# sash-a/es_pytorch

Hardware: AMD Instinct MI355X
Metric: env-steps/sec (whole node), Humanoid-v2 objective-ES (higher is better)
Workload: dtype bf16; 1 GPU; model=MLP(256, 256), env=Humanoid-v2, global_batch=1280, policies_per_gen=1280, episode_len=1000, seq_len=1000, objective=reward, parallelism=dp1, pair_rollout=True, eps_encoding=e4m3, noise_table_elems=250000000, n_params=166673

## Files before the change

es_pytorch_amd/core/engine.py:

```python
from __future__ import annotations

import time
from typing import List, Optional, Tuple

import numpy as np
import torch

from es_pytorch_amd import ops
from es_pytorch_amd.core.noisetable import NoiseTable
from es_pytorch_amd.core.policy import Policy
from es_pytorch_amd.envs.base import BatchedEnv
from es_pytorch_amd.nn.obstat import ObStat
from es_pytorch_amd.nn.optimizers import SGD, Adam, Optimizer
from es_pytorch_amd.parallel.comm import Comm
from es_pytorch_amd.rollout.results import RewardResult
from es_pytorch_amd.utils.novelty import novelty_batch
from es_pytorch_amd.utils.rankers import CenteredRanker, Ranker


def forward_perm(dims: List[int]) -> torch.Tensor:
    perm = []
    flat_off = 0
    for I, O in zip(dims[:-1], dims[1:]):
        w = np.arange(O * I, dtype=np.int64).reshape(O, I)
        perm.append((flat_off + w.T).reshape(-1))
        flat_off += O * I
        perm.append(np.arange(O, dtype=np.int64) + flat_off)
        flat_off += O
    return torch.from_numpy(np.concatenate(perm))


class _NoiselessResult(RewardResult):

    def __init__(self, reward: float, position, steps: int, ob_shape):
        super().__init__([reward], [float(position[0]), float(position[1]),
                                    float(position[2])] * 2,
                         np.zeros((1,) + tuple(ob_shape)), steps)


class GpuEngine:
    def __init__(self, cfg, comm: Comm, policy: Policy, nt: NoiseTable, env: BatchedEnv,
                 rs: np.random.RandomState, objective: str = "reward",
                 use_graph: bool = True, novelty_k: int = 10,
                 fused: Optional[bool] = None, rollout_mode: str = "step",
                 split_dyn: Optional[bool] = None,
                 pair_rollout: Optional[bool] = None,
                 eps_fp8: Optional[bool] = None,
                 weights_dtype: Optional[str] = None):
        self.rollout_mode = rollout_mode
        if weights_dtype is None:
            weights_dtype = cfg.general.get("weights_dtype", "bf16")
        if weights_dtype not in ("bf16", "fp32"):
            raise ValueError(f"weights_dtype must be 'bf16' or 'fp32', got "
                             f"{weights_dtype!r}")
        self.weights_dtype = weights_dtype
        self.fp32 = weights_dtype == "fp32"
        if self.fp32:
            for flag, val in (("pair_rollout", pair_rollout), ("eps_fp8", eps_fp8),
                              ("split_dyn", split_dyn)):
                if val is True:
                    raise ValueError(
                        f"{flag}=True is not available with weights_dtype='fp32' "
                        f"(the fp32 mode runs per-member fp32 rows only)")
            ignored = [k for k in ("pair_rollout", "eps_fp8", "split_dyn")
                       if bool(cfg.general.get(k, False))]
            if ignored and comm.rank == 0:
                import sys
                print(f"[engine] weights_dtype=fp32: ignoring {', '.join(ignored)} "
                      f"from the config (no fp32 variant)", file=sys.stderr)
            pair_rollout = eps_fp8 = split_dyn = False
        self.steps_per_launch = int(cfg.general.get("steps_per_launch", 1) or 1)
        self.cfg = cfg
        self.comm = comm
        self.policy = policy
        self.nt = nt
        self.env = env
        self.rs = rs
        self.objective = objective
        self.device = nt.noise.device
        self.use_graph = use_graph and self.device.type == "cuda"
        self.novelty_k = novelty_k
        self.archive: Optional[torch.Tensor] = None

        ppg = cfg.general.policies_per_gen
        assert ppg % comm.size == 0 and (ppg / comm.size) % 2 == 0, \
            "policies_per_gen must split into antithetic pairs per rank"
        self.pairs = int(ppg // comm.size // 2)
        self.eps = max(1, int(cfg.general.get("eps_per_policy", 1) or 1))
        self.M = 2 * self.pairs + 1
        self.B = self.M * self.eps
        assert env.batch == self.B, f"env batch {env.batch} != engine batch {self.B}"

        self.dims = policy._module.layer_dims()
        if len(self.dims) - 1 > 8:
            raise ValueError(
                f"model has {len(self.dims) - 1} layers; the fused HIP forward "
                f"supports at most 8 (ES_MAXL in ops/csrc/hip/mlp_core.h) — "
                f"reduce policy.layer_sizes or raise ES_MAXL and rebuild")
        if max(self.dims) > 2048:
            raise ValueError(
                f"widest layer is {max(self.dims)}; the fused HIP forward "
                f"supports at most 2048 (ES_MAXDIM in ops/csrc/hip/mlp_core.h) "
                f"— narrow policy.layer_sizes or raise ES_MAXDIM and rebuild")
        self.bins = int(getattr(policy._module, "bins", 0))
# ... 53 lines not shown
        self.rew_total = torch.zeros(self.B, dtype=torch.float32, device=d)
        self.member_steps = torch.zeros(self.B, dtype=torch.float32, device=d)
        self.behv = torch.zeros((self.B, 3), dtype=torch.float32, device=d)
        self.save_mask = torch.zeros(self.B, dtype=torch.float32, device=d)
        self.ob_sum = torch.zeros(D, dtype=torch.float64, device=d)
        self.ob_sumsq = torch.zeros(D, dtype=torch.float64, device=d)
        self.ob_count = torch.zeros((), dtype=torch.float64, device=d)
        self.obs_buf = torch.zeros((self.B, D), dtype=torch.float32, device=d)

        self.max_steps = int(cfg.env.max_steps)
        self.gen = 0
        self._graph: Optional[torch.cuda.CUDAGraph] = None
        self.timings = {}
        self._side = torch.cuda.Stream(self.device) if self.device.type == "cuda" else None
        self._offs_prefetched = False

        from es_pytorch_amd.envs.locomotion import SyntheticLocomotion
        self.fused = (isinstance(env, SyntheticLocomotion) and self.device.type == "cuda"
                      if fused is None else bool(fused))
        if self.fused:
            self.mo_sum = torch.zeros((self.B, D), dtype=torch.float32, device=d)
            self.mo_sumsq = torch.zeros((self.B, D), dtype=torch.float32, device=d)

        self.dyn_group = int(cfg.general.get("dyn_group", 5) or 5)
        want_split = bool(cfg.general.get("split_dyn", False)) if split_dyn is None \
            else bool(split_dyn)
        self.split_dyn = (want_split and self.fused and env.sdim % 8 == 0
                          and env.ac_dim <= 64 and self.dyn_group in (2, 4, 5, 8))
        if self.split_dyn:
            self.act_scratch = torch.empty(self.B * 64, dtype=torch.float32, device=d)

        fp8_possible = (bool(cfg.general.get("eps_fp8", False))
                        if eps_fp8 is None else bool(eps_fp8)) and \
            self.rollout_mode == "step" and self.steps_per_launch == 1 and \
            self._fp8_layout_ok(self.dims)
        if pair_rollout is not None:
            want_pair = bool(pair_rollout)
        else:
            gate_blocks = 256 if fp8_possible else 384
            want_pair = (bool(cfg.general.get("pair_rollout", False))
                         and self.pairs * self.eps >= gate_blocks)
        self.pair_rollout = (want_pair and self.fused and not self.split_dyn
                             and self.pairs >= 1)
        self._zero_off = torch.zeros(1, dtype=torch.int64, device=d)
        self._zero_sign = torch.zeros(1, dtype=torch.float32, device=d)
        want_fp8 = (bool(cfg.general.get("eps_fp8", False))
                    if eps_fp8 is None else bool(eps_fp8))
        self.eps_fp8 = fp8_possible and self.pair_rollout
        if want_fp8 and not self.eps_fp8 and comm.rank == 0:
            import sys
            print("[engine] eps_fp8 requested but unavailable for this "
                  "model/path — using bf16 eps rows", file=sys.stderr)
        if self.pair_rollout:
            self._theta_blob = torch.empty((2, self.row_stride), dtype=torch.bfloat16,
                                           device=d)
            self.theta_row = self._theta_blob[:1]
            eps_dt = torch.uint8 if self.eps_fp8 else torch.bfloat16
            self._eps_blob = torch.empty((self.pairs + 1, self.row_stride),
                                         dtype=eps_dt, device=d)
            self.eps_rows = self._eps_blob[:self.pairs]
            self._zeros_n = torch.zeros(self.n, dtype=torch.float32, device=d)
            self._one_signs = torch.ones(self.pairs, dtype=torch.float32, device=d)
        self._warned_host_ranker = False

    @staticmethod
    def _fp8_layout_ok(dims: List[int]) -> bool:
        off = 0
        for I, O in zip(dims[:-1], dims[1:]):
            vec = (O % 8 == 0) and (off % 8 == 0)
            if vec and (off + (I % 2) * O) % 16 != 0:
                return False
            off += I * O + O
        return True

    def _grad_qstd(self) -> float:
        return float(self.policy.std) if self.eps_fp8 else 0.0

    @property
    def numerics(self) -> dict:
        if self.pair_rollout:
            path, enc = "pair", "e4m3" if self.eps_fp8 else "bf16"
# ... 104 lines not shown
            ops.check(ops.hip().es_loco_step(*common, self._stream()), "es_loco_step")

    def _loco_episode(self, member_base: int, n_members: int, noiseless_from: int,
                      n_steps: Optional[int] = None, salt_base: int = 0,
                      weights_ptr: Optional[int] = None, wrow0: int = 0,
                      block_threads: int = 256):
        env = self.env
        goal_ptr = env.goal.data_ptr() if env.goal_conditioned else None
        fn, name = (ops.hip().es_loco_episode_f32, "es_loco_episode_f32") \
            if self.fp32 else (ops.hip().es_loco_episode, "es_loco_episode")
        ops.check(fn(
            self.weights.data_ptr() if weights_ptr is None else weights_ptr,
            self.obmean.data_ptr(), self.obstd.data_ptr(),
            self.dims_arr.ctypes.data, len(self.dims_arr), self.seed_dev.data_ptr(),
            self.max_steps if n_steps is None else n_steps,
            float(self.policy._module.ob_clip),
            self.acstd_dev.data_ptr(), self.row_stride,
            env.s.data_ptr(), env.pos.data_ptr(), goal_ptr,
            env.A_bf16.data_ptr(), env.B.data_ptr(), env.b0.data_ptr(),
            env.wv.data_ptr(), env.wa.data_ptr(), env.wy.data_ptr(), env.wh.data_ptr(),
            self.alive.data_ptr(), self.rew_total.data_ptr(),
            self.member_steps.data_ptr(), self.behv.data_ptr(),
            self.mo_sum.data_ptr(), self.mo_sumsq.data_ptr(),
            member_base, n_members, salt_base, wrow0, env.sdim, env.ac_dim,
            int(env.goal_conditioned), int(env.terminate_on_fall), noiseless_from,
            self.bins, self.eps, self.act_mode,
            float(env.leak), float(env.ctrl_cost), float(env.alive_bonus),
            float(env.fall_threshold), float(env.dt), int(block_threads),
            self._stream()), name)

    def _loco_pair_episode(self, n_steps: Optional[int] = None, salt_base: int = 0):
        env = self.env
        goal_ptr = env.goal.data_ptr() if env.goal_conditioned else None
        ops.check(ops.hip().es_loco_pair_episode(
            self.theta_row.data_ptr(), self.eps_rows.data_ptr(),
            self.obmean.data_ptr(), self.obstd.data_ptr(),
            self.dims_arr.ctypes.data, len(self.dims_arr),
            self.seed_dev.data_ptr(),
            float(self.policy._module.ob_clip), self.acstd_dev.data_ptr(),
            self.row_stride,
            env.s.data_ptr(), env.pos.data_ptr(), goal_ptr,
            env.A_bf16.data_ptr(), env.B.data_ptr(), env.b0.data_ptr(),
            env.wv.data_ptr(), env.wa.data_ptr(), env.wy.data_ptr(),
            env.wh.data_ptr(),
            self.alive.data_ptr(), self.rew_total.data_ptr(),
            self.member_steps.data_ptr(), self.behv.data_ptr(),
            self.mo_sum.data_ptr(), self.mo_sumsq.data_ptr(),
            self.pairs, env.sdim, env.ac_dim, int(env.goal_conditioned),
            int(env.terminate_on_fall), (self.M - 1) * self.eps, self.bins,
            self.eps, self.act_mode,
            float(env.leak), float(env.ctrl_cost), float(env.alive_bonus),
            float(env.fall_threshold), float(env.dt),
            self.max_steps if n_steps is None else int(n_steps), int(salt_base),
            self._stream()), "es_loco_pair_episode")

    def _loco_noiseless_episode(self):
        if self.pair_rollout:
            self._loco_episode((self.M - 1) * self.eps, self.eps, 0,
                               weights_ptr=self.theta_row.data_ptr(),
                               wrow0=self.M - 1, block_threads=512)
        else:
            self._loco_episode((self.M - 1) * self.eps, self.eps, 0,
                               block_threads=512)

    def _step_body(self, t: int):
        a = self._forward(self.obs_buf, salt=t + 1)
        ob, rew, done = self.env.step(a)
        alive = self.alive
        self.rew_total.add_(rew * alive)
        self.member_steps.add_(alive)
        am = alive.bool().unsqueeze(1)
        self.behv.copy_(torch.where(am, self.env.positions, self.behv))
        w = alive * self.save_mask
        self.ob_sum.add_((ob * w.unsqueeze(1)).sum(0).double())
        self.ob_sumsq.add_((ob * ob * w.unsqueeze(1)).sum(0).double())
        self.ob_count.add_(w.sum().double())
        self.alive.mul_(1.0 - done.float())
        self.obs_buf.copy_(ob)

    def _rollout_body(self):
        if self.fused and self.rollout_mode == "episode":
            main = torch.cuda.current_stream(self.device)
            self._side.wait_stream(main)
            with torch.cuda.stream(self._side):
                self._loco_noiseless_episode()
            if self.pair_rollout:
                self._loco_pair_episode()
# ... 2 lines not shown
            main.wait_stream(self._side)
            return
        if self.fused:
            main = torch.cuda.current_stream(self.device)
            self._side.wait_stream(main)
            with torch.cuda.stream(self._side):
                self._loco_noiseless_episode()
            k = self.steps_per_launch
            if k > 1:
                mm = (self.M - 1) * self.eps
                for t0 in range(0, self.max_steps, k):
                    n = min(k, self.max_steps - t0)
                    if self.pair_rollout:
                        self._loco_pair_episode(n_steps=n, salt_base=t0)
                    else:
                        self._loco_episode(0, mm, mm, n_steps=n, salt_base=t0)
            else:
                for t in range(self.max_steps):
                    self._loco_step(t)
            main.wait_stream(self._side)
        else:
            for t in range(self.max_steps):
                self._step_body(t)

    def _rollout(self):
        body = self._loco_step if self.fused else self._step_body
        if self.use_graph:
            if self._graph is None:
                s = torch.cuda.Stream(self.device)
                s.wait_stream(torch.cuda.current_stream(self.device))
                with torch.cuda.stream(s):
                    for t in range(3):
                        body(t)
                    if self.fused:
                        self._loco_noiseless_episode()
                torch.cuda.current_stream(self.device).wait_stream(s)
                self._reset_rollout_state()
                self.obs_buf.copy_(self.env.reset(self._gen_seed()))
                self._graph = torch.cuda.CUDAGraph()
                with torch.cuda.graph(self._graph):
                    self._rollout_body()
            self._graph.replay()
            return
        self._rollout_body()

    def _reset_rollout_state(self):
        self.alive.fill_(1.0)
        self.rew_total.zero_()
        self.member_steps.zero_()
        self.behv.zero_()
        self.ob_sum.zero_()
        self.ob_sumsq.zero_()
        self.ob_count.zero_()
        if self.fused:
            self.mo_sum.zero_()
            self.mo_sumsq.zero_()

    def _gen_seed(self) -> int:
        return (self.gen * 1000003 + self.comm.rank * 7919) & 0x7FFFFFFF

    def _member_rewards(self) -> torch.Tensor:
        return self.rew_total.view(self.M, self.eps).mean(1)

    def _member_behv(self) -> torch.Tensor:
        return self.behv.view(self.M, self.eps, 3)[:, -1]

# ... 269 lines not shown
```

es_pytorch_amd/ops/__init__.py:

```python
from __future__ import annotations

import ctypes
import os
import subprocess
from typing import Optional

_DIR = os.path.dirname(os.path.abspath(__file__))
_CPU_SO = os.path.join(_DIR, "_cpu_ops.so")
_HIP_SO = os.environ.get("ES_HIP_SO", os.path.join(_DIR, "_hip_ops.so"))

_cpu_lib: Optional[ctypes.CDLL] = None
_hip_lib: Optional[ctypes.CDLL] = None


class _BuildLock:

    def __init__(self, path: str):
        self.path = path + ".lock"
        self._fl = None

    def __enter__(self):
        try:
            from filelock import FileLock
            self._fl = FileLock(self.path)
# ... 110 lines not shown

def _bind_hip(lib):
    u64, i64, u32, i32, f32, p = (ctypes.c_uint64, ctypes.c_int64, ctypes.c_uint32,
                                  ctypes.c_int32, ctypes.c_float, ctypes.c_void_p)
    lib.es_noise_fill.argtypes = [p, i64, u64, u32, p]
    lib.es_pheno_bf16.argtypes = [p, p, p, p, p, i64, i64, i64, f32, p]
    lib.es_pheno_fp8.argtypes = [p, p, p, p, i32, i64, i64, i64, f32, p]
    lib.es_mlp_fwd.argtypes = [p, p, p, p, p, p, i32, p, u64, i32, f32, p, i64, i32,
                               i32, i32, i32, i32, p, p, p]
    lib.es_grad_gather.argtypes = [p, p, p, p, i64, i64, f32, p]
    lib.es_adam_step.argtypes = [p, p, p, p, i64, f32, f32, f32, f32, f32, f32, p]
    lib.es_sgd_step.argtypes = [p, p, p, i64, f32, f32, f32, f32, p]
    lib.es_loco_step.argtypes = [p, p, p, p, i32, p, u64, f32, p, i64,
                                 p, p, p, p, p, p, p, p, p, p,
                                 p, p, p, p, p, p,
                                 i32, i32, i32, i32, i32, i32, i32, i32, i32,
                                 f32, f32, f32, f32, f32, p]
    lib.es_loco_step_split.argtypes = [p, p, p, p, i32, p, u64, f32, p, i64,
                                       p, p, p, p, p, p, p, p, p, p,
                                       p, p, p, p, p, p,
                                       i32, i32, i32, i32, i32, i32, i32, i32, i32,
                                       f32, f32, f32, f32, f32, p, i32, p]
    lib.es_loco_pair_step.argtypes = [p, p, p, p, p, i32, p, u64, f32, p, i64,
                                      p, p, p, p, p, p, p, p, p, p,
                                      p, p, p, p, p, p,
                                      i32, i32, i32, i32, i32, i32, i32, i32, i32,
                                      f32, f32, f32, f32, f32, p]
    lib.es_loco_pair_step_fp8.argtypes = lib.es_loco_pair_step.argtypes
    lib.es_loco_pair_episode.argtypes = [p, p, p, p, p, i32, p, f32, p, i64,
                                         p, p, p, p, p, p, p, p, p, p,
                                         p, p, p, p, p, p,
                                         i32, i32, i32, i32, i32, i32, i32, i32, i32,
                                         f32, f32, f32, f32, f32, i32, i32, p]
    lib.es_loco_episode.argtypes = [p, p, p, p, i32, p, i32, f32, p, i64,
                                    p, p, p, p, p, p, p, p, p, p,
                                    p, p, p, p, p, p,
                                    i32, i32, i32, i32, i32, i32, i32, i32, i32, i32,
                                    i32, i32, f32, f32, f32, f32, f32, i32, p]
    lib.es_pheno_f32.argtypes = lib.es_pheno_bf16.argtypes
    lib.es_mlp_fwd_f32.argtypes = lib.es_mlp_fwd.argtypes
    lib.es_loco_step_f32.argtypes = lib.es_loco_step.argtypes
    lib.es_loco_episode_f32.argtypes = lib.es_loco_episode.argtypes
    for fn in ["es_pheno_f32", "es_mlp_fwd_f32", "es_loco_step_f32",
               "es_loco_episode_f32",
               "es_noise_fill", "es_pheno_bf16", "es_pheno_fp8", "es_mlp_fwd",
               "es_grad_gather", "es_adam_step", "es_sgd_step", "es_loco_step",
               "es_loco_step_split", "es_loco_pair_step", "es_loco_pair_step_fp8",
               "es_loco_pair_episode", "es_loco_episode"]:
        getattr(lib, fn).restype = i32


def check(ret: int, name: str):
    if ret != 0:
        raise RuntimeError(f"HIP op {name} failed with hipError_t={ret}")
```

es_pytorch_amd/ops/csrc/hip/rollout_loco.hip:

```cpp
#include "mlp_core.h"

struct LocoArgs {
  int S;
  int A;
  int D;
  int goal;
  int terminate;
  int noiseless_from;
  int bins;
  int act_mode;
  int eps;
  int wrow0;
  float leak, ctrl, alive_bonus, fall_thr, dt, ob_clip;
  int64_t row_stride;
};

struct LocoPtrs {
  const uint16_t* weights;
  const float *obmean, *obstd, *ac_std_dev;
  const uint64_t* seed_dev;
  float *s_glob, *pos;
  const float *goal, *Bm, *b0, *wv, *wa, *wy, *wh;
  const uint16_t* Am;
  float *alive, *rew_total, *member_steps, *behv, *mo_sum, *mo_sumsq;
// ... 112 lines not shown
      for (; i + 11 * PART < S; i += step4) {
        const uint4 n0 = ld(i + 8 * PART), n1 = ld(i + 9 * PART),
                    n2 = ld(i + 10 * PART), n3 = ld(i + 11 * PART);
        bf8_fma(c0, raws[i], acc);
        bf8_fma(c1, raws[i + PART], acc);
        bf8_fma(c2, raws[i + 2 * PART], acc);
        bf8_fma(c3, raws[i + 3 * PART], acc);
        c0 = d0; c1 = d1; c2 = d2; c3 = d3;
        d0 = n0; d1 = n1; d2 = n2; d3 = n3;
      }
      if (i < S) bf8_fma(c0, raws[i], acc);
      if (i + PART < S) bf8_fma(c1, raws[i + PART], acc);
      if (i + 2 * PART < S) bf8_fma(c2, raws[i + 2 * PART], acc);
      if (i + 3 * PART < S) bf8_fma(c3, raws[i + 3 * PART], acc);
      if (i + 4 * PART < S) bf8_fma(d0, raws[i + 4 * PART], acc);
      if (i + 5 * PART < S) bf8_fma(d1, raws[i + 5 * PART], acc);
      if (i + 6 * PART < S) bf8_fma(d2, raws[i + 6 * PART], acc);
      if (i + 7 * PART < S) bf8_fma(d3, raws[i + 7 * PART], acc);
      i += 8 * PART;
    }
    for (; i < S; i += PART) bf8_fma(ld(i), raws[i], acc);
#pragma unroll
    for (int q = 0; q < 8; ++q) partial[(ip * OCT + oi) * 8 + q] = acc[q];
  }
  __syncthreads();
}

#define ES_DYN_BM_BT 16

struct LocoBook {
  float px, py, gx, gy, rew_total, member_steps, ms0, ms1, mq0, mq1;
};

template <int NM>
__device__ __forceinline__ void loco_dyn_finish_n(
    const LocoArgs& la, const LocoPtrs& P, const int* b, const float* const* raws,
    const float* const* abuf, float* const* part, int tid, int nth) {
  const int S = la.S, A = la.A;
  float w_alive[NM];
  float *sb[NM], *ms[NM], *mq[NM];
#pragma unroll
  for (int m = 0; m < NM; ++m) {
    w_alive[m] = P.alive[b[m]];
    sb[m] = P.s_glob + (int64_t)b[m] * S;
    ms[m] = P.mo_sum + (int64_t)b[m] * la.D;
    mq[m] = P.mo_sumsq + (int64_t)b[m] * la.D;
  }
  const int wid = tid >> 6;
  const bool book = (tid & 63) == 0 && wid < NM;
  int bme = b[0];
  float alive_me = w_alive[0];
  float *part_me = part[0], *ms_me = ms[0], *mq_me = mq[0];
#pragma unroll
  for (int m = 1; m < NM; ++m)
    if (wid == m) {
      bme = b[m]; alive_me = w_alive[m];
      part_me = part[m]; ms_me = ms[m]; mq_me = mq[m];
    }
  LocoBook bk = {};
  if (book) {
    bk.px = P.pos[(int64_t)bme * 3 + 0];
    bk.py = P.pos[(int64_t)bme * 3 + 1];
    bk.rew_total = P.rew_total[bme];
    bk.member_steps = P.member_steps[bme];
    if (la.goal) {
      bk.gx = P.goal[(int64_t)bme * 2 + 0];
      bk.gy = P.goal[(int64_t)bme * 2 + 1];
      if (alive_me > 0.0f) {
        bk.ms0 = ms_me[S]; bk.ms1 = ms_me[S + 1];
        bk.mq0 = mq_me[S]; bk.mq1 = mq_me[S + 1];
      }
    }
  }

  float p0[NM], p1[NM], p2[NM], p3[NM];
#pragma unroll
  for (int m = 0; m < NM; ++m) p0[m] = p1[m] = p2[m] = p3[m] = 0.0f;
  {
    const bool oct8 = (S % 8 == 0);
    const int OCT = S >> 3;
    const int PART = oct8 ? nth / OCT : 0;
    for (int o = tid; o < S; o += nth) {
      const float b0o = P.b0[o], wvo = P.wv[o], wyo = P.wy[o], who = P.wh[o];
      float mso[NM], mqo[NM];
#pragma unroll
      for (int m = 0; m < NM; ++m)
        if (w_alive[m] > 0.0f) {
          mso[m] = ms[m][o];
          mqo[m] = mq[m][o];
        }
      float p[NM];
#pragma unroll
      for (int m = 0; m < NM; ++m) p[m] = b0o;
      if (oct8) {
        const int oo = o >> 3, j = o & 7;
        for (int pp = 0; pp < PART; ++pp)
#pragma unroll
          for (int m = 0; m < NM; ++m) p[m] += part[m][(pp * OCT + oo) * 8 + j];
      } else {
        for (int i = 0; i < S; ++i) {
          const float a = bf2f(P.Am[(int64_t)i * S + o]);
#pragma unroll
          for (int m = 0; m < NM; ++m) p[m] = fmaf(raws[m][i], a, p[m]);
        }
      }
      const float* bcol = P.Bm + o;
      int k0 = 0;
      for (; k0 + ES_DYN_BM_BT <= A; k0 += ES_DYN_BM_BT) {
        float bv[ES_DYN_BM_BT];
#pragma unroll
        for (int u = 0; u < ES_DYN_BM_BT; ++u) bv[u] = bcol[(int64_t)(k0 + u) * S];
#pragma unroll
        for (int u = 0; u < ES_DYN_BM_BT; ++u)
#pragma unroll
          for (int m = 0; m < NM; ++m) p[m] = fmaf(abuf[m][k0 + u], bv[u], p[m]);
      }
      if (k0 < A) {
        float bv[ES_DYN_BM_BT];
#pragma unroll
        for (int u = 0; u < ES_DYN_BM_BT - 1; ++u)
          if (k0 + u < A) bv[u] = bcol[(int64_t)(k0 + u) * S];
#pragma unroll
        for (int u = 0; u < ES_DYN_BM_BT - 1; ++u)
          if (k0 + u < A) {
#pragma unroll
            for (int m = 0; m < NM; ++m) p[m] = fmaf(abuf[m][k0 + u], bv[u], p[m]);
          }
      }
#pragma unroll
      for (int m = 0; m < NM; ++m) {
        const float sn = (1.0f - la.leak) * raws[m][o] + la.leak * tanhf(p[m]);
        sb[m][o] = sn;
        p0[m] = fmaf(sn, wvo, p0[m]);
        p1[m] = fmaf(sn, wyo, p1[m]);
        p2[m] = fmaf(sn, who, p2[m]);
        if (w_alive[m] > 0.0f) {
          ms[m][o] = mso[m] + sn;
          mq[m][o] = mqo[m] + sn * sn;
        }
      }
    }
    for (int j = tid; j < A; j += nth) {
      const float waj = P.wa[j];
#pragma unroll
      for (int m = 0; m < NM; ++m) {
        p0[m] = fmaf(0.5f * abuf[m][j], waj, p0[m]);
        p3[m] = fmaf(abuf[m][j], abuf[m][j], p3[m]);
      }
    }
  }
#pragma unroll
  for (int off = 32; off > 0; off >>= 1) {
#pragma unroll
    for (int m = 0; m < NM; ++m) {
      p0[m] += __shfl_down(p0[m], off);
      p1[m] += __shfl_down(p1[m], off);
      p2[m] += __shfl_down(p2[m], off);
      p3[m] += __shfl_down(p3[m], off);
    }
  }
  __syncthreads();
  if ((tid & 63) == 0) {
#pragma unroll
    for (int m = 0; m < NM; ++m) {
      part[m][wid * 4 + 0] = p0[m];
// ... 15 lines not shown
    }
    const float alive_old = alive_me;
    float rew;
    if (la.goal) {
      const float rx = bk.gx - bk.px;
      const float ry = bk.gy - bk.py;
      const float inv = 1.0f / (sqrtf(rx * rx + ry * ry) + 1e-6f);
      rew = vfwd * rx * inv + vy * ry * inv - la.ctrl * asq + la.alive_bonus;
    } else {
      rew = vfwd - la.ctrl * asq + la.alive_bonus;
    }
    const float px = bk.px + la.dt * vfwd;
    const float py = bk.py + la.dt * vy;
    P.pos[(int64_t)bme * 3 + 0] = px;
    P.pos[(int64_t)bme * 3 + 1] = py;
    P.pos[(int64_t)bme * 3 + 2] = h;
    const float done = (la.terminate && h < la.fall_thr) ? 1.0f : 0.0f;
    P.rew_total[bme] = bk.rew_total + rew * alive_old;
    P.member_steps[bme] = bk.member_steps + alive_old;
    if (alive_old > 0.0f) {
      P.behv[(int64_t)bme * 3 + 0] = px;
      P.behv[(int64_t)bme * 3 + 1] = py;
      P.behv[(int64_t)bme * 3 + 2] = h;
    }
    P.alive[bme] = alive_old * (1.0f - done);
    if (la.goal && alive_old > 0.0f) {
      const float rel0 = (bk.gx - px) * 0.1f;
      const float rel1 = (bk.gy - py) * 0.1f;
      ms_me[S] = bk.ms0 + rel0;
      mq_me[S] = bk.mq0 + rel0 * rel0;
      ms_me[S + 1] = bk.ms1 + rel1;
      mq_me[S + 1] = bk.mq1 + rel1 * rel1;
    }
  }
  __syncthreads();
}

__device__ __forceinline__ void loco_dyn_finish(
    const LocoArgs& la, const LocoPtrs& P, int b, const float* raws,
    const float* abuf, float* partial, int tid, int nth) {
  const int bs[1] = {b};
  const float* const rs[1] = {raws};
  const float* const as[1] = {abuf};
  float* const ps[1] = {partial};
  loco_dyn_finish_n<1>(la, P, bs, rs, as, ps, tid, nth);
}

__device__ __forceinline__ void loco_dyn_finish_pair(
    const LocoArgs& la, const LocoPtrs& P, int bp, int bm, const float* rawsP,
    const float* rawsM, const float* abufP, const float* abufM, float* partP,
    float* partM, int tid, int nth) {
  const int bs[2] = {bp, bm};
  const float* const rs[2] = {rawsP, rawsM};
  const float* const as[2] = {abufP, abufM};
  float* const ps[2] = {partP, partM};
  loco_dyn_finish_n<2>(la, P, bs, rs, as, ps, tid, nth);
}

template <typename WT = uint16_t>
__device__ __forceinline__ void loco_step_body(
    const MlpShape& sh, const LocoArgs& la, const LocoPtrs& P, int b, uint64_t salt,
    float* bufA, float* bufB, float* partial, float* raws, float* abuf) {
  loco_fwd_body<WT>(sh, la, P, b, salt, bufA, bufB, partial, raws, abuf);
  if (la.S % 8 == 0)
    loco_dyn_partials(P.Am, la.S, raws, partial, threadIdx.x, blockDim.x);
  loco_dyn_finish(la, P, b, raws, abuf, partial, threadIdx.x, blockDim.x);
}

#define ES_LOCO_CARVE(NTH)                                       \
  extern __shared__ __attribute__((aligned(16))) char smem[];    \
  float* bufA = reinterpret_cast<float*>(smem);                  \
  float* bufB = bufA + sh.maxdim;                                \
  float* partial = bufB + sh.maxdim;                             \
  float* raws = partial + (NTH) * 8;                             \
  float* abuf = raws + ((la.S + 3) & ~3);

__global__ void __launch_bounds__(256)
loco_step_kernel(MlpShape sh, LocoArgs la, LocoPtrs P, uint64_t salt) {
  ES_LOCO_CARVE(256);
  loco_step_body(sh, la, P, blockIdx.x, salt, bufA, bufB, partial, raws, abuf);
}

__global__ void __launch_bounds__(256)
loco_episode_kernel(MlpShape sh, LocoArgs la, LocoPtrs P, int member_base, int n_steps,
                    int salt_base) {
  ES_LOCO_CARVE(256);
  const int b = member_base + blockIdx.x;
  for (int t = 1; t <= n_steps; ++t)
    loco_step_body(sh, la, P, b, (uint64_t)(salt_base + t), bufA, bufB, partial, raws,
// ... 196 lines not shown
        uint4 d0 = ld(i + 4 * PART), d1 = ld(i + 5 * PART), d2 = ld(i + 6 * PART),
              d3 = ld(i + 7 * PART);
        for (; i + 11 * PART < S; i += step4) {
          const uint4 n0 = ld(i + 8 * PART), n1 = ld(i + 9 * PART),
                      n2 = ld(i + 10 * PART), n3 = ld(i + 11 * PART);
          fma2(c0, i);
          fma2(c1, i + PART);
          fma2(c2, i + 2 * PART);
          fma2(c3, i + 3 * PART);
          c0 = d0; c1 = d1; c2 = d2; c3 = d3;
          d0 = n0; d1 = n1; d2 = n2; d3 = n3;
        }
        if (i < S) fma2(c0, i);
        if (i + PART < S) fma2(c1, i + PART);
        if (i + 2 * PART < S) fma2(c2, i + 2 * PART);
        if (i + 3 * PART < S) fma2(c3, i + 3 * PART);
        if (i + 4 * PART < S) fma2(d0, i + 4 * PART);
        if (i + 5 * PART < S) fma2(d1, i + 5 * PART);
        if (i + 6 * PART < S) fma2(d2, i + 6 * PART);
        if (i + 7 * PART < S) fma2(d3, i + 7 * PART);
        i += 8 * PART;
      }
    }
    for (; i < S; i += PART) fma2(ld(i), i);
#pragma unroll
    for (int q = 0; q < 8; ++q) {
      partP[(ip * OCT + oi) * 8 + q] = accp[q];
      partM[(ip * OCT + oi) * 8 + q] = accm[q];
    }
  }
  __syncthreads();
}

template <typename EB, bool PIPE = true>
__device__ __forceinline__ void loco_pair_step_body(
    const MlpShape& sh, const LocoArgs& la, const LocoPtrs& P,
    const uint16_t* tb, const EB* eb, int bp, int bm, uint64_t salt,
    float* bufAp, float* bufAm, float* bufBp, float* bufBm, float* partial,
    float* rawsP, float* rawsM, float* abufP, float* abufM) {
  const int tid = threadIdx.x, nth = blockDim.x;
  loco_build_obs_pair(la, P, bp, bm, bufAp, bufAm, rawsP, rawsM, tid, nth);
  __syncthreads();
  float *ap, *am;
  if constexpr (sizeof(EB) == 1)
    mlp_layers_pair_fp8(tb, (const uint8_t*)eb, sh, bufAp, bufAm, bufBp, bufBm,
                        partial, tid, nth, 1, &ap, &am);
  else
    mlp_layers_pair(tb, (const uint16_t*)eb, sh, bufAp, bufAm, bufBp, bufBm,
                    partial, tid, nth, 1, &ap, &am);
  loco_decode_action(sh, la, P, bp, salt, ap, abufP, tid);
  loco_decode_action(sh, la, P, bm, salt, am, abufM, tid);
  __syncthreads();
  if (la.S % 8 == 0)
    loco_dyn_partials_pair<PIPE>(P.Am, la.S, rawsP, rawsM, partial, partial + 2048,
                                 tid, nth);
  loco_dyn_finish_pair(la, P, bp, bm, rawsP, rawsM, abufP, abufM, partial,
                       partial + 2048, tid, nth);
}

#define ES_LOCO_PAIR_CARVE()                                     \
  extern __shared__ __attribute__((aligned(16))) char smem[];    \
  float* bufAp = reinterpret_cast<float*>(smem);                 \
  float* bufAm = bufAp + sh.maxdim;                              \
  float* bufBp = bufAm + sh.maxdim;                              \
  float* bufBm = bufBp + sh.maxdim;                              \
  float* partial = bufBm + sh.maxdim;             \
  float* rawsP = partial + 2 * 256 * 8;                          \
  float* rawsM = rawsP + ((la.S + 3) & ~3);                      \
  float* abufP = rawsM + ((la.S + 3) & ~3);                      \
  float* abufM = abufP + 64;                                     \
  const int q = blockIdx.x;                                      \
  const int p = q / la.eps, e = q % la.eps;                      \
  const int bp = p * la.eps + e;                                 \
  const int bm = (n_pairs + p) * la.eps + e;                     \
  const auto* ebp = eb + (int64_t)p * la.row_stride;

__global__ void __launch_bounds__(256, 1)
loco_pair_step_kernel(MlpShape sh, LocoArgs la, LocoPtrs P, const uint16_t* tb,
                      const uint16_t* eb, int n_pairs, uint64_t salt) {
  ES_LOCO_PAIR_CARVE();
  loco_pair_step_body(sh, la, P, tb, ebp, bp, bm, salt, bufAp, bufAm, bufBp, bufBm,
                      partial, rawsP, rawsM, abufP, abufM);
}

__global__ void __launch_bounds__(256, 1)
loco_pair_step_fp8_kernel(MlpShape sh, LocoArgs la, LocoPtrs P, const uint16_t* tb,
                          const uint8_t* eb, int n_pairs, uint64_t salt) {
  ES_LOCO_PAIR_CARVE();
  loco_pair_step_body(sh, la, P, tb, ebp, bp, bm, salt, bufAp, bufAm, bufBp, bufBm,
                      partial, rawsP, rawsM, abufP, abufM);
}

__global__ void __launch_bounds__(256, 4)
loco_pair_episode_kernel(MlpShape sh, LocoArgs la, LocoPtrs P, const uint16_t* tb,
                         const uint16_t* eb, int n_pairs, int n_steps,
                         int salt_base) {
  ES_LOCO_PAIR_CARVE();
#pragma clang loop unroll(disable)
  for (int t = 1; t <= n_steps; ++t)
    loco_pair_step_body<uint16_t, false>(sh, la, P, tb, ebp, bp, bm, (uint64_t)(salt_base + t),
                        bufAp, bufAm, bufBp, bufBm, partial, rawsP, rawsM, abufP,
                        abufM);
}


struct LocoLaunch {
  MlpShape sh;
  LocoArgs la;
  LocoPtrs P;
};

static int loco_setup(LocoLaunch* L, const void* weights, const void* obmean,
                      const void* obstd, const int32_t* dims_host, int32_t ndims,
                      const void* seed_dev, float ob_clip, const void* ac_std_dev,
                      int64_t row_stride, void* s_glob, void* pos, const void* goal,
                      const void* Am, const void* Bm, const void* b0, const void* wv,
                      const void* wa, const void* wy, const void* wh, void* alive,
                      void* rew_total, void* member_steps, void* behv, void* mo_sum,
                      void* mo_sumsq, int32_t sdim, int32_t adim, int32_t goal_flag,
                      int32_t terminate, int32_t noiseless_from, int32_t bins,
                      int32_t eps, int32_t act_mode, float leak, float ctrl,
                      float alive_bonus, float fall_thr, float dt) {
  MlpShape* sh = &L->sh;
  int rc = mlp_shape_init(sh, dims_host, ndims, row_stride);
  if (rc) return rc;
  if (adim > 64 || sdim > ES_MAXDIM) return -103;
  if (sh->dims[0] != sdim + (goal_flag ? 2 : 0)) return -104;
  int out_dim = adim;
  if (bins > 1) out_dim = adim * bins;
  else if (act_mode == 2) out_dim = adim + 1;
  else if (act_mode == 3) out_dim = adim * 2;
  if (sh->dims[sh->n_layers] != out_dim) return -105;
  LocoArgs* la = &L->la;
  la->S = sdim; la->A = adim; la->D = sh->dims[0]; la->goal = goal_flag;
  la->terminate = terminate; la->noiseless_from = noiseless_from; la->bins = bins;
// ... 150 lines not shown
  LocoLaunch L;
  int rc = loco_setup(&L, nullptr, obmean, obstd, dims_host, ndims, seed_dev, ob_clip,
                      ac_std_dev, row_stride, s_glob, pos, goal, Am, Bm, b0, wv, wa, wy,
                      wh, alive, rew_total, member_steps, behv, mo_sum, mo_sumsq, sdim,
                      adim, goal_flag, terminate, noiseless_from, bins, eps, act_mode,
                      leak, ctrl, alive_bonus, fall_thr, dt);
  return rc ? rc
            : loco_launch_pair(loco_pair_step_fp8_kernel, L, theta_row, eps_rows,
                               n_pairs, stream, salt);
}

extern "C" int es_loco_pair_episode(
    const void* theta_row, const void* eps_rows, const void* obmean,
    const void* obstd, const int32_t* dims_host, int32_t ndims, const void* seed_dev,
    float ob_clip, const void* ac_std_dev, int64_t row_stride,
    void* s_glob, void* pos, const void* goal, const void* Am, const void* Bm,
    const void* b0, const void* wv, const void* wa, const void* wy, const void* wh,
    void* alive, void* rew_total, void* member_steps, void* behv, void* mo_sum,
    void* mo_sumsq, int32_t n_pairs, int32_t sdim, int32_t adim, int32_t goal_flag,
    int32_t terminate, int32_t noiseless_from, int32_t bins, int32_t eps,
    int32_t act_mode, float leak, float ctrl, float alive_bonus, float fall_thr,
    float dt, int32_t n_steps, int32_t salt_base, void* stream) {
  LocoLaunch L;
  int rc = loco_setup(&L, nullptr, obmean, obstd, dims_host, ndims, seed_dev, ob_clip,
                      ac_std_dev, row_stride, s_glob, pos, goal, Am, Bm, b0, wv, wa, wy,
                      wh, alive, rew_total, member_steps, behv, mo_sum, mo_sumsq, sdim,
                      adim, goal_flag, terminate, noiseless_from, bins, eps, act_mode,
                      leak, ctrl, alive_bonus, fall_thr, dt);
  return rc ? rc
            : loco_launch_pair(loco_pair_episode_kernel, L, theta_row, eps_rows, n_pairs,
                               stream, n_steps, salt_base);
}

extern "C" int es_loco_episode(const void* weights, const void* obmean, const void* obstd,
                               const int32_t* dims_host, int32_t ndims, const void* seed_dev,
                               int32_t n_steps, float ob_clip, const void* ac_std_dev,
                               int64_t row_stride,
                               void* s_glob, void* pos, const void* goal, const void* Am,
                               const void* Bm, const void* b0, const void* wv,
                               const void* wa, const void* wy, const void* wh, void* alive,
                               void* rew_total, void* member_steps, void* behv,
                               void* mo_sum, void* mo_sumsq, int32_t member_base,
                               int32_t n_members, int32_t salt_base, int32_t wrow0,
                               int32_t sdim, int32_t adim,
                               int32_t goal_flag, int32_t terminate, int32_t noiseless_from,
                               int32_t bins, int32_t eps, int32_t act_mode, float leak,
                               float ctrl, float alive_bonus, float fall_thr, float dt,
                               int32_t block_threads, void* stream) {
  LocoLaunch L;
  int rc = loco_setup(&L, weights, obmean, obstd, dims_host, ndims, seed_dev, ob_clip,
                      ac_std_dev, row_stride, s_glob, pos, goal, Am, Bm, b0, wv, wa, wy,
                      wh, alive, rew_total, member_steps, behv, mo_sum, mo_sumsq, sdim,
                      adim, goal_flag, terminate, noiseless_from, bins, eps, act_mode,
                      leak, ctrl, alive_bonus, fall_thr, dt);
  return rc ? rc
            : loco_launch_episode<uint16_t>(L, n_steps, member_base, n_members, salt_base,
                                            wrow0, block_threads, stream);
}

extern "C" int es_loco_step_f32(
    const void* weights, const void* obmean, const void* obstd,
    const int32_t* dims_host, int32_t ndims, const void* seed_dev, uint64_t salt,
    float ob_clip, const void* ac_std_dev, int64_t row_stride, void* s_glob, void* pos,
    const void* goal, const void* Am, const void* Bm, const void* b0, const void* wv,
    const void* wa, const void* wy, const void* wh, void* alive, void* rew_total,
    void* member_steps, void* behv, void* mo_sum, void* mo_sumsq, int32_t n_pop,
// ... 34 lines not shown
```

Measured before the change: 22.37 million env-steps/s.

## Add multi-step fp8 pair-rollout chunk kernel and auto-enable it for small populations

Adds an fp8-eps pair rollout kernel that runs many env steps per launch, with optional carry of the next observation between steps. The engine now allows eps_fp8 with steps_per_launch > 1 and, when steps_per_launch is unset and pairs*eps fits within four blocks per CU, sets it to 50 so one launch covers 50 steps. The aim is to cut per-step kernel launch and graph overhead. The cost is a larger kernel held under a fixed occupancy bound, plus opaque-register hints that may affect register pressure. Graph warmup now also runs the chunked episode path.

```diff
diff --git a/es_pytorch_amd/core/engine.py b/es_pytorch_amd/core/engine.py
--- a/es_pytorch_amd/core/engine.py
+++ b/es_pytorch_amd/core/engine.py
@@ -16,6 +16,9 @@
 from es_pytorch_amd.rollout.results import RewardResult
 from es_pytorch_amd.utils.novelty import novelty_batch
 from es_pytorch_amd.utils.rankers import CenteredRanker, Ranker
+
+FP8_PAIR_STEPS_PER_LAUNCH = 50
+FP8_PAIR_CHUNK_BLOCKS_PER_CU = 4
 
 
 def forward_perm(dims: List[int]) -> torch.Tensor:
@@ -69,7 +72,9 @@
                 print(f"[engine] weights_dtype=fp32: ignoring {', '.join(ignored)} "
                       f"from the config (no fp32 variant)", file=sys.stderr)
             pair_rollout = eps_fp8 = split_dyn = False
-        self.steps_per_launch = int(cfg.general.get("steps_per_launch", 1) or 1)
+        spl = cfg.general.get("steps_per_launch", None)
+        self._steps_per_launch_auto = not spl
+        self.steps_per_launch = int(spl or 1)
         self.cfg = cfg
         self.comm = comm
         self.policy = policy
@@ -189,7 +194,6 @@
 
         fp8_possible = (bool(cfg.general.get("eps_fp8", False))
                         if eps_fp8 is None else bool(eps_fp8)) and \
-            self.rollout_mode == "step" and self.steps_per_launch == 1 and \
             self._fp8_layout_ok(self.dims)
         if pair_rollout is not None:
             want_pair = bool(pair_rollout)
@@ -204,6 +208,11 @@
         want_fp8 = (bool(cfg.general.get("eps_fp8", False))
                     if eps_fp8 is None else bool(eps_fp8))
         self.eps_fp8 = fp8_possible and self.pair_rollout
+        if self.eps_fp8 and self._steps_per_launch_auto and d.type == "cuda":
+            slots = FP8_PAIR_CHUNK_BLOCKS_PER_CU * \
+                torch.cuda.get_device_properties(d).multi_processor_count
+            if self.pairs * self.eps <= slots:
+                self.steps_per_launch = FP8_PAIR_STEPS_PER_LAUNCH
         if want_fp8 and not self.eps_fp8 and comm.rank == 0:
             import sys
             print("[engine] eps_fp8 requested but unavailable for this "
@@ -374,7 +383,9 @@
     def _loco_pair_episode(self, n_steps: Optional[int] = None, salt_base: int = 0):
         env = self.env
         goal_ptr = env.goal.data_ptr() if env.goal_conditioned else None
-        ops.check(ops.hip().es_loco_pair_episode(
+        fn, name = (ops.hip().es_loco_pair_episode_fp8, "es_loco_pair_episode_fp8") \
+            if self.eps_fp8 else (ops.hip().es_loco_pair_episode, "es_loco_pair_episode")
+        ops.check(fn(
             self.theta_row.data_ptr(), self.eps_rows.data_ptr(),
             self.obmean.data_ptr(), self.obstd.data_ptr(),
             self.dims_arr.ctypes.data, len(self.dims_arr),
@@ -394,7 +405,7 @@
             float(env.leak), float(env.ctrl_cost), float(env.alive_bonus),
             float(env.fall_threshold), float(env.dt),
             self.max_steps if n_steps is None else int(n_steps), int(salt_base),
-            self._stream()), "es_loco_pair_episode")
+            self._stream()), name)
 
     def _loco_noiseless_episode(self):
         if self.pair_rollout:
@@ -463,6 +474,13 @@
                 with torch.cuda.stream(s):
                     for t in range(3):
                         body(t)
+                    if self.fused and (self.rollout_mode == "episode"
+                                       or self.steps_per_launch > 1):
+                        if self.pair_rollout:
+                            self._loco_pair_episode(n_steps=2)
+                        else:
+                            mm = (self.M - 1) * self.eps
+                            self._loco_episode(0, mm, mm, n_steps=2)
                     if self.fused:
                         self._loco_noiseless_episode()
                 torch.cuda.current_stream(self.device).wait_stream(s)
diff --git a/es_pytorch_amd/ops/__init__.py b/es_pytorch_amd/ops/__init__.py
--- a/es_pytorch_amd/ops/__init__.py
+++ b/es_pytorch_amd/ops/__init__.py
@@ -166,6 +166,8 @@
                                          p, p, p, p, p, p,
                                          i32, i32, i32, i32, i32, i32, i32, i32, i32,
                                          f32, f32, f32, f32, f32, i32, i32, p]
+    lib.es_loco_pair_episode_fp8.argtypes = lib.es_loco_pair_episode.argtypes
+    lib.es_loco_pair_episode_fp8_config.argtypes = [i32, i32]
     lib.es_loco_episode.argtypes = [p, p, p, p, i32, p, i32, f32, p, i64,
                                     p, p, p, p, p, p, p, p, p, p,
                                     p, p, p, p, p, p,
@@ -180,7 +182,8 @@
                "es_noise_fill", "es_pheno_bf16", "es_pheno_fp8", "es_mlp_fwd",
                "es_grad_gather", "es_adam_step", "es_sgd_step", "es_loco_step",
                "es_loco_step_split", "es_loco_pair_step", "es_loco_pair_step_fp8",
-               "es_loco_pair_episode", "es_loco_episode"]:
+               "es_loco_pair_episode", "es_loco_pair_episode_fp8",
+               "es_loco_pair_episode_fp8_config", "es_loco_episode"]:
         getattr(lib, fn).restype = i32
 
 
diff --git a/es_pytorch_amd/ops/csrc/hip/rollout_loco.hip b/es_pytorch_amd/ops/csrc/hip/rollout_loco.hip
--- a/es_pytorch_amd/ops/csrc/hip/rollout_loco.hip
+++ b/es_pytorch_amd/ops/csrc/hip/rollout_loco.hip
@@ -168,10 +168,11 @@
   float px, py, gx, gy, rew_total, member_steps, ms0, ms1, mq0, mq1;
 };
 
-template <int NM>
+template <int NM, bool CARRY = false>
 __device__ __forceinline__ void loco_dyn_finish_n(
     const LocoArgs& la, const LocoPtrs& P, const int* b, const float* const* raws,
-    const float* const* abuf, float* const* part, int tid, int nth) {
+    const float* const* abuf, float* const* part, int tid, int nth,
+    float* const* obs = nullptr, bool carry = false) {
   const int S = la.S, A = la.A;
   float w_alive[NM];
   float *sb[NM], *ms[NM], *mq[NM];
@@ -208,6 +209,18 @@
       }
     }
   }
+  float* obs_me = nullptr;
+  float gmean0 = 0.0f, gmean1 = 0.0f, gsd0 = 1.0f, gsd1 = 1.0f;
+  if constexpr (CARRY) {
+    if (carry && la.goal && book) {
+      obs_me = obs[0];
+#pragma unroll
+      for (int m = 1; m < NM; ++m)
+        if (wid == m) obs_me = obs[m];
+      gmean0 = P.obmean[S]; gmean1 = P.obmean[S + 1];
+      gsd0 = P.obstd[S]; gsd1 = P.obstd[S + 1];
+    }
+  }
 
   float p0[NM], p1[NM], p2[NM], p3[NM];
 #pragma unroll
@@ -218,6 +231,9 @@
     const int PART = oct8 ? nth / OCT : 0;
     for (int o = tid; o < S; o += nth) {
       const float b0o = P.b0[o], wvo = P.wv[o], wyo = P.wy[o], who = P.wh[o];
+      float omean = 0.0f, osd = 1.0f;
+      if constexpr (CARRY)
+        if (carry) { omean = P.obmean[o]; osd = P.obstd[o]; }
       float mso[NM], mqo[NM];
 #pragma unroll
       for (int m = 0; m < NM; ++m)
@@ -267,6 +283,11 @@
       for (int m = 0; m < NM; ++m) {
         const float sn = (1.0f - la.leak) * raws[m][o] + la.leak * tanhf(p[m]);
         sb[m][o] = sn;
+        if constexpr (CARRY)
+          if (carry) {
+            const_cast<float*>(raws[m])[o] = sn;
+            obs[m][o] = fclampf((sn - omean) / osd, -la.ob_clip, la.ob_clip);
+          }
         p0[m] = fmaf(sn, wvo, p0[m]);
         p1[m] = fmaf(sn, wyo, p1[m]);
         p2[m] = fmaf(sn, who, p2[m]);
@@ -348,6 +369,14 @@
       ms_me[S + 1] = bk.ms1 + rel1;
       mq_me[S + 1] = bk.mq1 + rel1 * rel1;
     }
+    if constexpr (CARRY) {
+      if (carry && la.goal) {
+        const float rel0 = (bk.gx - px) * 0.1f;
+        const float rel1 = (bk.gy - py) * 0.1f;
+        obs_me[S] = fclampf((rel0 - gmean0) / gsd0, -la.ob_clip, la.ob_clip);
+        obs_me[S + 1] = fclampf((rel1 - gmean1) / gsd1, -la.ob_clip, la.ob_clip);
+      }
+    }
   }
   __syncthreads();
 }
@@ -362,15 +391,18 @@
   loco_dyn_finish_n<1>(la, P, bs, rs, as, ps, tid, nth);
 }
 
+template <bool CARRY = false>
 __device__ __forceinline__ void loco_dyn_finish_pair(
     const LocoArgs& la, const LocoPtrs& P, int bp, int bm, const float* rawsP,
     const float* rawsM, const float* abufP, const float* abufM, float* partP,
-    float* partM, int tid, int nth) {
+    float* partM, int tid, int nth, float* obsP = nullptr, float* obsM = nullptr,
+    bool carry = false) {
   const int bs[2] = {bp, bm};
   const float* const rs[2] = {rawsP, rawsM};
   const float* const as[2] = {abufP, abufM};
   float* const ps[2] = {partP, partM};
-  loco_dyn_finish_n<2>(la, P, bs, rs, as, ps, tid, nth);
+  float* const os[2] = {obsP, obsM};
+  loco_dyn_finish_n<2, CARRY>(la, P, bs, rs, as, ps, tid, nth, os, carry);
 }
 
 template <typename WT = uint16_t>
@@ -633,15 +665,18 @@
   __syncthreads();
 }
 
-template <typename EB, bool PIPE = true>
+template <typename EB, bool PIPE = true, bool CARRY = false>
 __device__ __forceinline__ void loco_pair_step_body(
     const MlpShape& sh, const LocoArgs& la, const LocoPtrs& P,
     const uint16_t* tb, const EB* eb, int bp, int bm, uint64_t salt,
     float* bufAp, float* bufAm, float* bufBp, float* bufBm, float* partial,
-    float* rawsP, float* rawsM, float* abufP, float* abufM) {
-  const int tid = threadIdx.x, nth = blockDim.x;
-  loco_build_obs_pair(la, P, bp, bm, bufAp, bufAm, rawsP, rawsM, tid, nth);
-  __syncthreads();
+    float* rawsP, float* rawsM, float* abufP, float* abufM, int tid,
+    bool have = false, bool keep = false) {
+  const int nth = blockDim.x;
+  if (!(CARRY && have)) {
+    loco_build_obs_pair(la, P, bp, bm, bufAp, bufAm, rawsP, rawsM, tid, nth);
+    __syncthreads();
+  }
   float *ap, *am;
   if constexpr (sizeof(EB) == 1)
     mlp_layers_pair_fp8(tb, (const uint8_t*)eb, sh, bufAp, bufAm, bufBp, bufBm,
@@ -655,8 +690,8 @@
   if (la.S % 8 == 0)
     loco_dyn_partials_pair<PIPE>(P.Am, la.S, rawsP, rawsM, partial, partial + 2048,
                                  tid, nth);
-  loco_dyn_finish_pair(la, P, bp, bm, rawsP, rawsM, abufP, abufM, partial,
-                       partial + 2048, tid, nth);
+  loco_dyn_finish_pair<CARRY>(la, P, bp, bm, rawsP, rawsM, abufP, abufM, partial,
+                              partial + 2048, tid, nth, bufAp, bufAm, keep);
 }
 
 #define ES_LOCO_PAIR_CARVE()                                     \
@@ -681,7 +716,7 @@
                       const uint16_t* eb, int n_pairs, uint64_t salt) {
   ES_LOCO_PAIR_CARVE();
   loco_pair_step_body(sh, la, P, tb, ebp, bp, bm, salt, bufAp, bufAm, bufBp, bufBm,
-                      partial, rawsP, rawsM, abufP, abufM);
+                      partial, rawsP, rawsM, abufP, abufM, threadIdx.x);
 }
 
 __global__ void __launch_bounds__(256, 1)
@@ -689,7 +724,7 @@
                           const uint8_t* eb, int n_pairs, uint64_t salt) {
   ES_LOCO_PAIR_CARVE();
   loco_pair_step_body(sh, la, P, tb, ebp, bp, bm, salt, bufAp, bufAm, bufBp, bufBm,
-                      partial, rawsP, rawsM, abufP, abufM);
+                      partial, rawsP, rawsM, abufP, abufM, threadIdx.x);
 }
 
 __global__ void __launch_bounds__(256, 4)
@@ -701,7 +736,37 @@
   for (int t = 1; t <= n_steps; ++t)
     loco_pair_step_body<uint16_t, false>(sh, la, P, tb, ebp, bp, bm, (uint64_t)(salt_base + t),
                         bufAp, bufAm, bufBp, bufBm, partial, rawsP, rawsM, abufP,
-                        abufM);
+                        abufM, threadIdx.x);
+}
+
+#define ES_OPAQUE_S(x) asm volatile("" : "+s"(x))
+#define ES_OPAQUE_V(x) asm volatile("" : "+v"(x))
+template <int MINB, bool CARRY>
+__global__ void __launch_bounds__(256, MINB)
+loco_pair_chunk_fp8_kernel(MlpShape sh, LocoArgs la, LocoPtrs Pk, const uint16_t* tb,
+                           const uint8_t* eb, int n_pairs, int n_steps, int salt_base) {
+  ES_LOCO_PAIR_CARVE();
+  LocoPtrs P = Pk;
+  int bpl = bp, bml = bm;
+  int tid = threadIdx.x;
+  const bool oct8 = (la.S % 8 == 0);
+#pragma clang loop unroll(disable)
+  for (int t = 1; t <= n_steps; ++t) {
+    ES_OPAQUE_S(P.weights); ES_OPAQUE_S(P.obmean); ES_OPAQUE_S(P.obstd);
+    ES_OPAQUE_S(P.ac_std_dev); ES_OPAQUE_S(P.seed_dev); ES_OPAQUE_S(P.s_glob);
+    ES_OPAQUE_S(P.pos); ES_OPAQUE_S(P.goal); ES_OPAQUE_S(P.Bm); ES_OPAQUE_S(P.b0);
+    ES_OPAQUE_S(P.wv); ES_OPAQUE_S(P.wa); ES_OPAQUE_S(P.wy); ES_OPAQUE_S(P.wh);
+    ES_OPAQUE_S(P.Am); ES_OPAQUE_S(P.alive); ES_OPAQUE_S(P.rew_total);
+    ES_OPAQUE_S(P.member_steps); ES_OPAQUE_S(P.behv); ES_OPAQUE_S(P.mo_sum);
+    ES_OPAQUE_S(P.mo_sumsq);
+    ES_OPAQUE_S(tb); ES_OPAQUE_S(ebp); ES_OPAQUE_S(bpl); ES_OPAQUE_S(bml);
+    ES_OPAQUE_V(tid);
+    ES_OPAQUE_S(la.leak); ES_OPAQUE_S(la.ob_clip);
+    loco_pair_step_body<uint8_t, true, CARRY>(
+        sh, la, P, tb, ebp, bpl, bml, (uint64_t)(salt_base + t), bufAp, bufAm, bufBp,
+        bufBm, partial, rawsP, rawsM, abufP, abufM, tid, oct8 && t > 1,
+        oct8 && t < n_steps);
+  }
 }
 
 
@@ -918,6 +983,49 @@
                                stream, n_steps, salt_base);
 }
 
+#define ES_CHUNK_FP8_MIN_BLOCKS 4
+#define ES_CHUNK_FP8_CARRY 0
+static int g_chunk_fp8_min_blocks = ES_CHUNK_FP8_MIN_BLOCKS;
+static int g_chunk_fp8_carry = ES_CHUNK_FP8_CARRY;
+
+extern "C" int es_loco_pair_episode_fp8_config(int32_t min_blocks, int32_t carry) {
+  if (min_blocks == 0) {
+    min_blocks = ES_CHUNK_FP8_MIN_BLOCKS;
+    carry = ES_CHUNK_FP8_CARRY;
+  }
+  if (min_blocks != 3 && min_blocks != 4) return -108;
+  g_chunk_fp8_min_blocks = min_blocks;
+  g_chunk_fp8_carry = carry != 0;
+  return 0;
+}
+
+extern "C" int es_loco_pair_episode_fp8(
+    const void* theta_row, const void* eps_rows, const void* obmean,
+    const void* obstd, const int32_t* dims_host, int32_t ndims, const void* seed_dev,
+    float ob_clip, const void* ac_std_dev, int64_t row_stride,
+    void* s_glob, void* pos, const void* goal, const void* Am, const void* Bm,
+    const void* b0, const void* wv, const void* wa, const void* wy, const void* wh,
+    void* alive, void* rew_total, void* member_steps, void* behv, void* mo_sum,
+    void* mo_sumsq, int32_t n_pairs, int32_t sdim, int32_t adim, int32_t goal_flag,
+    int32_t terminate, int32_t noiseless_from, int32_t bins, int32_t eps,
+    int32_t act_mode, float leak, float ctrl, float alive_bonus, float fall_thr,
+    float dt, int32_t n_steps, int32_t salt_base, void* stream) {
+  LocoLaunch L;
+  int rc = loco_setup(&L, nullptr, obmean, obstd, dims_host, ndims, seed_dev, ob_clip,
+                      ac_std_dev, row_stride, s_glob, pos, goal, Am, Bm, b0, wv, wa, wy,
+                      wh, alive, rew_total, member_steps, behv, mo_sum, mo_sumsq, sdim,
+                      adim, goal_flag, terminate, noiseless_from, bins, eps, act_mode,
+                      leak, ctrl, alive_bonus, fall_thr, dt);
+  if (rc) return rc;
+  const bool four = g_chunk_fp8_min_blocks == 4, carry = g_chunk_fp8_carry != 0;
+  auto* kern = four ? (carry ? loco_pair_chunk_fp8_kernel<4, true>
+                             : loco_pair_chunk_fp8_kernel<4, false>)
+                    : (carry ? loco_pair_chunk_fp8_kernel<3, true>
+                             : loco_pair_chunk_fp8_kernel<3, false>);
+  return loco_launch_pair(kern, L, theta_row, eps_rows, n_pairs, stream, n_steps,
+                          salt_base);
+}
+
 extern "C" int es_loco_episode(const void* weights, const void* obmean, const void* obstd,
                                const int32_t* dims_host, int32_t ndims, const void* seed_dev,
                                int32_t n_steps, float ob_clip, const void* ac_std_dev,
```

New measurement: 23.14 million env-steps/s (median of 6 runs). +3.5%, better.
